# chagmgang/distributed_reinforcement_learning

Measured on AMD Instinct MI355X. Metric: learner env-frames/sec (whole node), IMPALA deep-conv 84x84x4, higher is better.
Workload: dtype bf16; 1 GPU; model=impala deep-conv 84x84x4 + LSTM256 V-trace, global_batch=32, seq_len=20, parallelism=dp1, num_action=18

## Files before the change

distributed_reinforcement_learning_amd/ops/hip/bind.cpp:

```cpp

#include <torch/extension.h>
#include <ATen/hip/HIPContext.h>
#include <hip/hip_runtime.h>

#include <algorithm>
#include <array>
#include <tuple>

#include "drla_kernels.h"

namespace {

hipStream_t cur_stream() {
  return at::hip::getCurrentHIPStream().stream();
}

void check_gpu_contig(const torch::Tensor& t, const char* name) {
  TORCH_CHECK(t.is_cuda(), name, " must be on the GPU");
  TORCH_CHECK(t.is_contiguous(), name, " must be contiguous");
}

template <typename... Ts>
void check_all_gpu_contig(const char* what, const Ts&... ts) {
  (check_gpu_contig(ts, what), ...);
// ... 139 lines not shown
                    slab.scalar_type() == torch::kBFloat16 &&
                    slab.size(0) == batch && slab.size(1) >= row &&
                    slab.stride(1) == 1 && slab.stride(0) >= slab.size(1),
                "out_slab must be a row-major [batch, >= ho*wo*co] bf16 "
                "buffer");
    out_n_stride = slab.stride(0);
    out = slab.as_strided(
        {batch, cfg.ho, cfg.wo, cfg.co},
        {out_n_stride, (long long)cfg.wo * cfg.co, cfg.co, 1});
  } else {
    out = torch::empty({batch, cfg.ho, cfg.wo, cfg.co},
                       in.options().dtype(torch::kBFloat16));
  }
  const dim3 grid(conv_m_tiles(batch * cfg.ho * cfg.wo));
  torch::Tensor x_stash;
  unsigned char* stashp = nullptr;
  if (stash_input) {
    TORCH_CHECK(layer <= 1, "input stash is a u8-layer feature");
    TORCH_CHECK((in.numel() % 16) == 0, "stash wants 16-divisible bytes");
    x_stash = torch::empty_like(in);
    stashp = x_stash.data_ptr<uint8_t>();
  }
  if (layer <= 1) {
    hipLaunchKernelGGL(kConvFwdU8[layer], grid, dim3(DRLA_CONV_BLOCK), 0,
                       cur_stream(), in.data_ptr<uint8_t>(), BF16P(w),
                       BF16P(bias), BF16PM(out), batch, stashp, slotp,
                       in_dist);
  } else {
    hipLaunchKernelGGL(kConvFwdBf16[layer - 2], grid, dim3(DRLA_CONV_BLOCK),
                       0, cur_stream(), BF16P(in), BF16P(w), BF16P(bias),
                       BF16PM(out), batch, out_n_stride);
  }
  return {out, x_stash};
}

static torch::Tensor& dbias_slot_buf(const torch::Tensor& like,
                                     int64_t slot_id) {
  static torch::Tensor bufs[4];
  TORCH_CHECK(slot_id >= 0 && slot_id < 4, "bad slot id");
  if (!bufs[slot_id].defined()) {
    bufs[slot_id] =
        torch::zeros({DRLA_DBIAS_SLOTS * DRLA_DBIAS_STRIDE},
                     like.options().dtype(torch::kFloat));
  }
  return bufs[slot_id];
}

torch::Tensor relu_mask_bwd(torch::Tensor dy, torch::Tensor y, int64_t CO,
                            int64_t slot_id) {
  TORCH_CHECK(dy.is_cuda() && y.is_cuda(), "dy and y must be on GPU");
  TORCH_CHECK(dy.numel() == y.numel() && dy.size(0) == y.size(0),
              "dy and y must hold the same rows");
  long long row_elems = dy.numel() / std::max<int64_t>(dy.size(0), 1);
  auto n_stride_of = [row_elems](const torch::Tensor& t, const char* name) {
    if (t.is_contiguous()) return row_elems;
    for (int d = 1; d < t.dim(); ++d) {
      TORCH_CHECK(t.stride(d - 1) >= t.stride(d), name, " must be row-major");
    }
    TORCH_CHECK(t.stride(t.dim() - 1) == 1 && t.stride(0) >= row_elems &&
                    row_elems % 8 == 0 && t.stride(0) % 8 == 0 &&
                    t.storage_offset() % 8 == 0,
                name, " view must be inner-contiguous and 16 B aligned");
    for (int d = 1; d + 1 < t.dim(); ++d) {
      TORCH_CHECK(t.stride(d) == t.size(d + 1) * t.stride(d + 1), name,
                  " inner dims must be contiguous");
    }
    return (long long)t.stride(0);
  };
  const long long n_stride = n_stride_of(dy, "dy");
  const long long y_n_stride = n_stride_of(y, "y");
  auto out = torch::empty(dy.sizes(), dy.options());
  auto& slots = dbias_slot_buf(dy, slot_id);
  const long long n = dy.numel();
  TORCH_CHECK(n % 8 == 0, "relu_mask_bwd wants numel % 8 == 0");
  int grid = drla_grid(n / 8);
  if (grid > 640) grid = 640;
  hipLaunchKernelGGL(drla_relu_mask_bwd, dim3(grid), dim3(DRLA_BLOCK),
                     0, cur_stream(), BF16P(dy), BF16P(y), BF16PM(out),
                     slots.data_ptr<float>(), n, (int)CO, n_stride,
                     row_elems, y_n_stride);
  return out;
}

std::tuple<torch::Tensor, torch::Tensor> conv_wgrad(int layer,
                                                    torch::Tensor in,
                                                    torch::Tensor dy) {
  check_gpu_contig(in, "in");
  check_gpu_contig(dy, "dy");
  const auto& cfg = conv_layer(layer);
  const int batch = in.size(0);
  const int K = cfg.kh * cfg.kw * cfg.ci;
  static int split_env = [] {
    const char* e = getenv("DRLA_WGRAD_SPLIT");
    return e ? atoi(e) : 0;
  }();
  const int split = split_env ? split_env : ((layer <= 1) ? 512 : 64);
  static torch::Tensor scratch_cache[4];
  if (!scratch_cache[layer].defined()) {
    scratch_cache[layer] =
        torch::zeros({K, cfg.co}, dy.options().dtype(torch::kFloat));
  }
  auto scratch = scratch_cache[layer];
  const dim3 grid((K + DRLA_CONV_WGRAD_BK - 1) / DRLA_CONV_WGRAD_BK, split);
  if (layer <= 1) {
    hipLaunchKernelGGL(kConvWgradU8[layer], grid, dim3(DRLA_CONV_BLOCK), 0,
                       cur_stream(), in.data_ptr<uint8_t>(), BF16P(dy),
                       scratch.data_ptr<float>(), batch);
  } else {
    hipLaunchKernelGGL(kConvWgradBf16[layer - 2], grid,
                       dim3(DRLA_CONV_BLOCK), 0, cur_stream(), BF16P(in),
                       BF16P(dy), scratch.data_ptr<float>(), batch);
  }
  auto dw = torch::empty({cfg.co, K}, dy.options().dtype(torch::kBFloat16));
  auto dbias = torch::empty({cfg.co}, dy.options().dtype(torch::kBFloat16));
  auto& slots = dbias_slot_buf(dy, layer);
  hipLaunchKernelGGL(drla_wgrad_finalize,
                     dim3(drla_grid((long long)K * cfg.co)),
                     dim3(DRLA_BLOCK), 0, cur_stream(),
                     scratch.data_ptr<float>(), BF16PM(dw), K, cfg.co,
                     slots.data_ptr<float>(), BF16PM(dbias));
  return {dw, dbias};
}

torch::Tensor conv_dgrad(int layer, torch::Tensor dy, torch::Tensor w) {
  check_gpu_contig(dy, "dy");
  check_gpu_contig(w, "w");
  TORCH_CHECK(layer == 2 || layer == 3, "dgrad only for l2/l3");
  const auto& cfg = conv_layer(layer);
  const int batch = dy.size(0);
  auto dx = torch::empty({batch, cfg.hi, cfg.wi, cfg.ci},
                         dy.options().dtype(torch::kBFloat16));
  if (layer == 2) {
    const int grid_c = conv_m_tiles(batch * (cfg.hi / 2) * (cfg.wi / 2));
    hipLaunchKernelGGL(drla_conv_dgrad_l2, dim3(grid_c, 4),
                       dim3(DRLA_CONV_BLOCK), 0, cur_stream(), BF16P(dy),
                       BF16P(w), BF16PM(dx), batch);
  } else {
    hipLaunchKernelGGL(drla_conv_dgrad_l3,
                       dim3(conv_m_tiles(batch * cfg.hi * cfg.wi)),
                       dim3(DRLA_CONV_BLOCK), 0, cur_stream(), BF16P(dy),
                       BF16P(w), BF16PM(dx), batch);
  }
  return dx;
}

std::tuple<torch::Tensor, torch::Tensor> dqn_loss_fwd(
    torch::Tensor main_q, torch::Tensor next_main, torch::Tensor next_tgt,
    torch::Tensor actions, torch::Tensor rewards, torch::Tensor discounts,
    torch::Tensor weights) {
  check_all_gpu_contig("dqn_loss input", main_q, next_main, next_tgt,
                       actions, rewards, discounts, weights);
  TORCH_CHECK(actions.scalar_type() == torch::kInt, "actions must be i32");
  const int B = main_q.size(0), A = main_q.size(1);
  const DualPtr mq = dual_ptr(main_q);
  auto fopt = rewards.options().dtype(torch::kFloat);
  auto loss = torch::zeros({1}, fopt);
  auto td = torch::empty({B}, fopt);
  hipLaunchKernelGGL(
      drla_dqn_loss_fwd, dim3((B + 255) / 256), dim3(256), 0, cur_stream(),
      mq.bf16, mq.f32, next_main.data_ptr<float>(), next_tgt.data_ptr<float>(),
      actions.data_ptr<int>(), rewards.data_ptr<float>(),
      discounts.data_ptr<float>(), weights.data_ptr<float>(),
      loss.data_ptr<float>(), td.data_ptr<float>(), B, A);
  return {loss, td};
}

torch::Tensor dqn_loss_bwd(torch::Tensor td, torch::Tensor actions,
                           torch::Tensor weights, torch::Tensor gloss,
                           int64_t A, bool want_bf16) {
  check_all_gpu_contig("dqn_loss bwd input", td, actions, weights, gloss);
  const int B = td.numel();
  auto dmq = torch::empty(
      {B, A},
      td.options().dtype(want_bf16 ? torch::kBFloat16 : torch::kFloat));
  const DualPtr out = dual_ptr(dmq);
  hipLaunchKernelGGL(
      drla_dqn_loss_bwd, dim3(((long long)B * A + 255) / 256), dim3(256), 0,
      cur_stream(), td.data_ptr<float>(), actions.data_ptr<int>(),
      weights.data_ptr<float>(), gloss.data_ptr<float>(), out.bf16, out.f32,
// ... 915 lines not shown
}

void rmsprop_step_t(torch::Tensor p, torch::Tensor g, torch::Tensor ms,
                    double clip, torch::Tensor lr_buf, double rho,
                    double eps) {
  check_all_gpu_contig("rmsprop tensor", p, g, ms, lr_buf);
  const long long n = p.numel();
  torch::Tensor norm_buf;
  if (clip > 0) {
    norm_buf = sq_norm(g);
  } else {
    norm_buf = torch::zeros({1}, p.options());
  }
  hipLaunchKernelGGL(drla_rmsprop_step, dim3(drla_grid(n)), dim3(DRLA_BLOCK),
                     0, cur_stream(), p.data_ptr<float>(),
                     g.data_ptr<float>(), ms.data_ptr<float>(),
                     norm_buf.data_ptr<float>(), static_cast<float>(clip),
                     lr_buf.data_ptr<float>(), static_cast<float>(rho),
                     static_cast<float>(eps), n);
}

void rmsprop_step(torch::Tensor p, torch::Tensor g, torch::Tensor ms,
                  double clip, double lr, double rho, double eps) {
  auto lr_buf = torch::full({1}, lr, p.options());
  rmsprop_step_t(p, g, ms, clip, lr_buf, rho, eps);
}

void adam_step_t(torch::Tensor p, torch::Tensor g, torch::Tensor m,
                 torch::Tensor v, double clip, torch::Tensor lr_buf,
                 double beta1, double beta2, double eps) {
  check_all_gpu_contig("adam tensor", p, g, m, v, lr_buf);
  const long long n = p.numel();
  torch::Tensor norm_buf;
  if (clip > 0) {
    norm_buf = sq_norm(g);
  } else {
    norm_buf = torch::zeros({1}, p.options());
  }
  hipLaunchKernelGGL(drla_adam_step, dim3(drla_grid(n)), dim3(DRLA_BLOCK), 0,
                     cur_stream(), p.data_ptr<float>(), g.data_ptr<float>(),
                     m.data_ptr<float>(), v.data_ptr<float>(),
                     norm_buf.data_ptr<float>(), static_cast<float>(clip),
                     lr_buf.data_ptr<float>(), static_cast<float>(beta1),
                     static_cast<float>(beta2), static_cast<float>(eps), n);
}

void adam_step(torch::Tensor p, torch::Tensor g, torch::Tensor m,
               torch::Tensor v, double clip, double lr_t, double beta1,
               double beta2, double eps) {
  auto lr_buf = torch::full({1}, lr_t, p.options());
  adam_step_t(p, g, m, v, clip, lr_buf, beta1, beta2, eps);
}

}

PYBIND11_MODULE(TORCH_EXTENSION_NAME, m) {
  m.def("normalize_frames_f32", &normalize_frames_f32,
        "uint8 frames -> float32/255 (K11)");
  m.def("normalize_frames_bf16", &normalize_frames_bf16,
        "uint8 frames -> bf16/255 (K11)");
  m.def("vtrace_scan", &vtrace_scan, "fused V-trace reverse scan (K5)");
  m.def("_set_lr_slot", &set_lr_slot,
        "write the learning rate and the input-slot word in one launch");
  m.def("vtrace_loss_fwd", &vtrace_loss_fwd,
        "fused IMPALA loss pipeline forward (K5+K7+K13); nofill: ticketed "
        "fixed-order loss sums, no zero-fill; stash_actions: also returns "
        "a copy of actions made in-kernel",
        py::arg("logits"), py::arg("value"), py::arg("mu"),
        py::arg("actions"), py::arg("rewards"), py::arg("done"),
        py::arg("gamma"), py::arg("clip_mode"), py::arg("c_bl"),
        py::arg("c_ent"), py::arg("nofill") = false,
        py::arg("stash_actions") = false, py::arg("slot") = py::none(),
        py::arg("slot_dist") = std::vector<int64_t>{});
  m.def("vtrace_loss_bwd", &vtrace_loss_bwd,
        "fused IMPALA loss pipeline backward (closed form)");
  m.def("mfma_probe", &mfma_probe, "16x16x32 bf16 MFMA layout probe");
  m.def("conv_fwd", &conv_fwd,
        "MFMA implicit-GEMM conv fwd, fused normalize+bias+ReLU (K1)",
        py::arg("layer"), py::arg("x"), py::arg("w"), py::arg("bias"),
        py::arg("stash_input"), py::arg("out_slab") = py::none(),
        py::arg("slot") = py::none(),
        py::arg("slot_dist") = std::vector<int64_t>{});
  m.def("conv_wgrad", &conv_wgrad, "MFMA conv weight gradient (K1 bwd)");
  m.def("conv_dgrad", &conv_dgrad, "MFMA conv data gradient (K1 bwd)");
  m.def("relu_mask_bwd", &relu_mask_bwd,
        "fused-ReLU backward mask + bias gradient");
  m.def("dqn_loss_fwd", &dqn_loss_fwd,
        "fused double-DQN target + IS-weighted TD loss (K8)");
  m.def("dqn_loss_bwd", &dqn_loss_bwd, "closed-form K8 backward");
  m.def("a2c_loss_fwd", &a2c_loss_fwd, "fused A2C loss fwd (K6)");
  m.def("a2c_loss_bwd", &a2c_loss_bwd, "fused A2C loss bwd (K6)");
  m.def("r2d2_loss_fwd", &r2d2_loss_fwd,
        "fused R2D2 sequence-TD tail fwd (K9; n_step > 1 or "
        "priority_eta >= 0 selects the n-step kernel)",
        py::arg("mq"), py::arg("tq"), py::arg("actions"), py::arg("rewards"),
        py::arg("done"), py::arg("weights"), py::arg("gamma"),
        py::arg("clip_mode"), py::arg("n_step") = 1,
        py::arg("priority_eta") = -1.0);
  m.def("dhead_train_fwd", &dhead_train_fwd,
        "grad-carrying dueling head fwd (R2D2 trained window)");
  m.def("dhead_train_bwd", &dhead_train_bwd,
        "grad-carrying dueling head bwd chain + weight grads");
  m.def("dueling_head_fwd", &dueling_head_fwd,
        "no-grad dueling head over the post-burn-in window");
  m.def("r2d2_loss_bwd", &r2d2_loss_bwd,
        "fused R2D2 sequence-TD tail bwd (K9)");
  m.def("per_update", &per_update, "GPU PER segment-tree batched update");
  m.def("per_sample", &per_sample, "GPU PER stratified sample descent");
  m.def("multi_gather", &multi_gather,
        "one-kernel replay batch gather (all fields)");
  m.def("per_rebuild", &per_rebuild,
        "GPU PER interior-sum rebuild (float32 drift repair)");
  m.def("embed_bwd", &embed_bwd,
        "action-embedding table gradient (K2 backward)");
  m.def("lstm_tail_fwd", &lstm_tail_fwd, "fused LSTM gate tail fwd (K3)",
        py::arg("gates"), py::arg("c_prev"), py::arg("forget_bias"),
        py::arg("stash_c") = false, py::arg("slot") = py::none(),
        py::arg("slot_dist") = std::vector<int64_t>{});
  m.def("lstm_tail_bwd", &lstm_tail_bwd, "fused LSTM gate tail bwd (K3)");
  m.def("mlp_heads_fwd", &mlp_heads_fwd,
        "fused policy+value MLP heads forward (K4)",
        py::arg("h"), py::arg("weights"), py::arg("biases"), py::arg("A"),
        py::arg("want_bwd_bufs") = false);
  m.def("mlp_heads_bwd", &mlp_heads_bwd,
        "fused heads dgrad chain + ReLU masks + bias grads (K4 bwd)",
        py::arg("dlogits"), py::arg("dvalue"), py::arg("stash"),
        py::arg("weights"), py::arg("A"), py::arg("ws") = py::none());
  m.def("embed_mlp_fwd", &embed_mlp_fwd,
        "fused action-embedding MLP forward (K2)",
        py::arg("pa"), py::arg("table"), py::arg("b1"), py::arg("w2"),
        py::arg("b2"), py::arg("stash_idx") = false,
        py::arg("want_w2t") = false, py::arg("xh_slab") = py::none(),
        py::arg("emb_col") = 0, py::arg("h") = py::none(),
        py::arg("slot") = py::none(),
        py::arg("slot_dist") = std::vector<int64_t>{});
  m.def("embed_mlp_bwd", &embed_mlp_bwd,
        "fused action-embedding MLP backward (K2 bwd)",
        py::arg("dy"), py::arg("out"), py::arg("a1"), py::arg("w2"),
        py::arg("idx"), py::arg("A"), py::arg("w2t") = py::none(),
        py::arg("fuse_scatter") = false);
  m.def("mlp_heads_pack_wt", &mlp_heads_pack_wt,
        "one-kernel transposed-weight pack for the heads dgrad");
  m.def("mlp_heads_wgrad", &mlp_heads_wgrad,
        "all six head wgrads (dW = dz^T @ act) in one MFMA launch");
  m.def("lstm_seq_train_fwd", &lstm_seq_train_fwd,
        "grad-carrying whole-sequence LSTM forward (K3 seq, R2D2 train)");
  m.def("lstm_seq_train_bwd", &lstm_seq_train_bwd,
        "whole-sequence LSTM backward (one kernel over the recurrence)");
  m.def("lstm_seq_fwd", &lstm_seq_fwd,
        "whole no-grad LSTM unroll in one kernel (K3 seq / burn-in)");
  m.def("sq_norm", &sq_norm, "squared L2 norm of a flat tensor (K12)");
  m.def("grad_gather", &grad_gather,
        "one-kernel scattered-grad -> flat bucket pack (K12b)");
  m.def("rmsprop_step", &rmsprop_step,
        "fused global-norm-clip + TF-RMSProp update (K12)");
  m.def("rmsprop_step_t", &rmsprop_step_t,
        "RMSProp update with device-tensor lr (hipGraph-safe)");
  m.def("adam_step", &adam_step,
        "fused global-norm-clip + TF-Adam update (K12)");
  m.def("adam_step_t", &adam_step_t,
        "Adam update with device-tensor lr_t (hipGraph-safe)");
  m.def("sq_norm_bf16", &sq_norm_bf16, "squared L2 norm of a bf16 tensor");
  m.def("rmsprop_step_bf16_t", &rmsprop_step_bf16_t,
        "bf16-model/fp32-master RMSProp (K12, mixed precision)");
  m.def("adam_step_bf16_t", &adam_step_bf16_t,
        "bf16-model/fp32-master Adam (K12, mixed precision)");
// ... 2 lines not shown
```

distributed_reinforcement_learning_amd/ops/hip/conv.hip:

```cpp

#include "drla_kernels.h"

#define CONV_KERNEL \
  extern "C" __global__ __launch_bounds__(DRLA_CONV_BLOCK) void

extern "C" __global__ void drla_mfma_probe(const bf16raw* __restrict__ A,
                                           const bf16raw* __restrict__ B,
                                           float* __restrict__ D) {
  const int l = threadIdx.x;
  bf16x8 a_frag, b_frag;
  for (int e = 0; e < 8; ++e) {
    a_frag[e] = (short)A[(l & 15) * 32 + ((l >> 4) * 8 + e)];
    b_frag[e] = (short)B[((l >> 4) * 8 + e) * 16 + (l & 15)];
  }
  f32x4 acc = {0.f, 0.f, 0.f, 0.f};
  acc = __builtin_amdgcn_mfma_f32_16x16x32_bf16(a_frag, b_frag, acc, 0, 0, 0);
  for (int r = 0; r < 4; ++r) {
    D[((l >> 4) * 4 + r) * 16 + (l & 15)] = acc[r];
  }
}


template <typename IN_T, int CI, int CO, int KH, int KW, int STRIDE, int HI,
          int WI, int HO, int WO>
__device__ void conv_fwd_impl(const IN_T* __restrict__ in,
                              const bf16raw* __restrict__ w,
                              const bf16raw* __restrict__ bias,
                              bf16raw* __restrict__ out,
                              int batch,
                              IN_T* __restrict__ x_stash = nullptr,
                              long long out_n_stride = 0) {
  constexpr int K = KH * KW * CI;
  constexpr int BM = DRLA_CONV_BM;
  constexpr int BK = 32;
  constexpr int APAD = 8;
  constexpr int NFRAG = CO / 16;
  const int M = batch * HO * WO;

  __shared__ bf16raw Abuf[BM][BK + APAD];
  __shared__ bf16raw Bbuf[CO][BK + APAD];
  __shared__ float BiasBuf[CO];

  const int tid = threadIdx.x;
  const int wave = tid / 64;
  const int lane = tid % 64;
  const int row0 = blockIdx.x * BM;

  if (tid < CO) BiasBuf[tid] = drla_bf16_to_f32(bias[tid]);

  f32x4 acc[2][NFRAG];
  for (int mi = 0; mi < 2; ++mi)
    for (int ni = 0; ni < NFRAG; ++ni)
      acc[mi][ni] = {0.f, 0.f, 0.f, 0.f};

  const int a_row = tid >> 1;
  const int a_k0 = (tid & 1) * 16;
  const int gm = row0 + a_row;
  const int n_idx = gm / (HO * WO);
  const int rem = gm - n_idx * (HO * WO);
  const int ho = rem / WO;
  const int wo = rem - ho * WO;
  const long long in_base =
      ((long long)n_idx * HI + ho * STRIDE) * WI + wo * STRIDE;

  unsigned int ra4u_0, ra4u_1, ra4u_2, ra4u_3;
  unsigned int ra1u[4];
  bf16x8 rab0 = {0, 0, 0, 0, 0, 0, 0, 0}, rab1 = rab0;
  uint4 rbw4;
  uint2 rbw2;
  constexpr int THREADS_PER_CO = DRLA_CONV_BLOCK / CO;
  constexpr int KCHUNK = BK / THREADS_PER_CO;
  const int b_co = tid / THREADS_PER_CO;
  const int b_kpart = (tid % THREADS_PER_CO) * KCHUNK;

  auto load_chunk = [&](int k0) {
    if (gm < M) {
      if constexpr (CI == 4) {
        const int kk = k0 + a_k0;
        const int kh = kk / (KW * CI);
        const int kw = (kk - kh * KW * CI) / CI;
        const uint4 packed = *reinterpret_cast<const uint4*>(
            in + (in_base + (long long)kh * WI + kw) * CI);
        ra4u_0 = packed.x; ra4u_1 = packed.y;
        ra4u_2 = packed.z; ra4u_3 = packed.w;
// ... 162 lines not shown
    bf16raw* __restrict__ out, float* __restrict__ dbias_slots,
    long long n, int CO, long long n_stride, long long row_elems,
    long long y_n_stride) {
  const long long n8 = n / 8;
  const long long stride = gridDim.x * (long long)blockDim.x;
  long long i = blockIdx.x * (long long)blockDim.x + threadIdx.x;
  const int tid = threadIdx.x;
  float acc[8] = {0, 0, 0, 0, 0, 0, 0, 0};
  const uint4* dy4 = reinterpret_cast<const uint4*>(dy);
  const uint4* y4 = reinterpret_cast<const uint4*>(y);
  uint4* out4 = reinterpret_cast<uint4*>(out);
#define DRLA_RM_LANE(dw, yw, ow, a0, a1)                              \
  {                                                                   \
    const bf16raw d0 = (bf16raw)((dw) & 0xFFFF);                      \
    const bf16raw d1 = (bf16raw)((dw) >> 16);                         \
    const bf16raw m0 =                                                \
        (drla_bf16_to_f32((bf16raw)((yw) & 0xFFFF)) > 0.0f) ? d0 : (bf16raw)0; \
    const bf16raw m1 =                                                \
        (drla_bf16_to_f32((bf16raw)((yw) >> 16)) > 0.0f) ? d1 : (bf16raw)0;    \
    (ow) = ((unsigned int)m1 << 16) | m0;                             \
    (a0) += drla_bf16_to_f32(m0);                                              \
    (a1) += drla_bf16_to_f32(m1);                                              \
  }
  const long long row8 = row_elems / 8;
  const bool strided = (n_stride != row_elems);
  const bool y_strided = (y_n_stride != row_elems);
  for (; i < n8; i += stride) {
    long long si = i, yi = i;
    if (strided || y_strided) {
      const long long r = i / row8;
      const long long c8 = i - r * row8;
      if (strided) si = (r * n_stride) / 8 + c8;
      if (y_strided) yi = (r * y_n_stride) / 8 + c8;
    }
    const uint4 dv = dy4[si];
    const uint4 yv = y4[yi];
    uint4 ov;
    DRLA_RM_LANE(dv.x, yv.x, ov.x, acc[0], acc[1]);
    DRLA_RM_LANE(dv.y, yv.y, ov.y, acc[2], acc[3]);
    DRLA_RM_LANE(dv.z, yv.z, ov.z, acc[4], acc[5]);
    DRLA_RM_LANE(dv.w, yv.w, ov.w, acc[6], acc[7]);
    out4[i] = ov;
  }
#undef DRLA_RM_LANE
  __shared__ float red[DRLA_BLOCK * 8];
  for (int e = 0; e < 8; ++e) red[tid * 8 + e] = acc[e];
  __syncthreads();
  if (tid < CO) {
    const int g = tid / 8;
    const int e = tid % 8;
    float s = 0.0f;
    for (int t = g; t < DRLA_BLOCK; t += CO / 8) s += red[t * 8 + e];
    atomicAdd(&dbias_slots[(blockIdx.x & (DRLA_DBIAS_SLOTS - 1)) *
                               DRLA_DBIAS_STRIDE +
                           tid], s);
  }
}

extern "C" __global__ void drla_wgrad_finalize(
    float* __restrict__ scratch, bf16raw* __restrict__ dw, int K,
    int CO, float* __restrict__ dbias_slots,
    bf16raw* __restrict__ dbias) {
  if (dbias_slots && blockIdx.x == 0 && (int)threadIdx.x < CO) {
    float s = 0.0f;
    for (int t = 0; t < DRLA_DBIAS_SLOTS; ++t) {
      s += dbias_slots[t * DRLA_DBIAS_STRIDE + threadIdx.x];
      dbias_slots[t * DRLA_DBIAS_STRIDE + threadIdx.x] = 0.0f;
    }
    dbias[threadIdx.x] = drla_f32_to_bf16(s);
  }
  long long i = blockIdx.x * (long long)blockDim.x + threadIdx.x;
  const long long total = (long long)K * CO;
  const long long stride = gridDim.x * (long long)blockDim.x;
  for (; i < total; i += stride) {
    const int co = i / K;
    const int k = i - (long long)co * K;
    const long long si = (long long)k * CO + co;
    dw[i] = drla_f32_to_bf16(scratch[si]);
    scratch[si] = 0.0f;
  }
}


template <typename IN_T, int CI, int CO, int KH, int KW, int STRIDE, int HI,
          int WI, int HO, int WO>
__device__ void conv_wgrad_impl(const IN_T* __restrict__ in,
                                const bf16raw* __restrict__ dy,
                                float* __restrict__ scratch,
                                int batch) {
  constexpr int K = KH * KW * CI;
  constexpr int BKM = 64;
  constexpr int BKK = DRLA_CONV_WGRAD_BK;
  constexpr int PAD = 8;
  constexpr int NFRAG = CO / 16;
  constexpr int CO_PER_T = (CO * 32) / DRLA_CONV_BLOCK;
  const int M = batch * HO * WO;

  __shared__ bf16raw Am[2][BKK][BKM + PAD];
  __shared__ bf16raw BmT[2][CO][BKM + PAD];

  const int tid = threadIdx.x;
  const int wave = tid / 64;
  const int lane = tid % 64;
  const int k_row0 = blockIdx.x * BKK;

  f32x4 acc[NFRAG];
  for (int ni = 0; ni < NFRAG; ++ni) acc[ni] = {0.f, 0.f, 0.f, 0.f};

  const int m_per_split = (M + gridDim.y - 1) / gridDim.y;
  const int m_begin = blockIdx.y * m_per_split;
  const int m_end = min(M, m_begin + m_per_split);

  const int a_m = tid >> 2;
  const int a_k = (tid & 3) * 16;
  long long a_off0 = 0, a_off1 = 0;
  long long a_offc[16];
  if constexpr (CI == 4) {
    const int kb = k_row0 + a_k;
    const int kh = kb / (KW * CI);
    a_off0 = (long long)kh * WI + (kb - kh * KW * CI) / CI;
  } else if constexpr (CI == 1) {
    static_assert(K % BKK == 0,
                  "CI==1 contiguous row staging requires K % BKK == 0");
#pragma unroll
    for (int t = 0; t < 16; ++t) {
      const int k2 = k_row0 + a_k + t;
      const int kh = k2 / KW;
      a_offc[t] = (k2 < K) ? (long long)kh * WI + (k2 - kh * KW) : -1;
    }
  } else {
    const int kk0 = k_row0 + a_k;
    const int kh0 = kk0 / (KW * CI);
    const int kwci0 = kk0 - kh0 * KW * CI;
    a_off0 = (kk0 < K)
        ? ((long long)kh0 * WI + kwci0 / CI) * CI + (kwci0 % CI) : -1;
    const int kk1 = kk0 + 8;
    const int kh1 = kk1 / (KW * CI);
    const int kwci1 = kk1 - kh1 * KW * CI;
    a_off1 = (kk1 < K)
        ? ((long long)kh1 * WI + kwci1 / CI) * CI + (kwci1 % CI) : -1;
  }
  const int b_lm0 = tid / (CO / CO_PER_T);
  const int b_co0 = (tid % (CO / CO_PER_T)) * CO_PER_T;

  unsigned int ra4u_0, ra4u_1, ra4u_2, ra4u_3;
  unsigned int ra1u[4];
  bf16x8 rab0 = {0, 0, 0, 0, 0, 0, 0, 0}, rab1 = rab0;
  bf16x8 rb8_0 = rab0, rb8_1 = rab0;
  uint2 rb4_0 = {0, 0}, rb4_1 = {0, 0};
  bool a_live = false, b_live0 = false, b_live1 = false;

  auto load_chunk = [&](int m0) {
    const int m = m0 + a_m;
    a_live = (m < m_end);
    if (a_live) {
      const int n_idx = m / (HO * WO);
      const int rem = m - n_idx * (HO * WO);
      const int ho = rem / WO;
      const int wo = rem - ho * WO;
      const long long base =
          ((long long)n_idx * HI + ho * STRIDE) * WI + wo * STRIDE;
      if constexpr (CI == 4) {
        const uint4 packed = *reinterpret_cast<const uint4*>(
            in + (base + a_off0) * CI);
        ra4u_0 = packed.x; ra4u_1 = packed.y;
        ra4u_2 = packed.z; ra4u_3 = packed.w;
      } else if constexpr (CI == 1) {
#pragma unroll
        for (int rrow = 0; rrow < 2; ++rrow) {
          const unsigned char* src = in + base + a_offc[rrow * 8];
          ra1u[rrow * 2 + 0] = *reinterpret_cast<const unsigned int*>(src);
          ra1u[rrow * 2 + 1] =
              *reinterpret_cast<const unsigned int*>(src + 4);
        }
      } else {
        const bf16raw* inb = reinterpret_cast<const bf16raw*>(in);
        if (a_off0 >= 0) {
          rab0 = *reinterpret_cast<const bf16x8*>(inb + base * CI + a_off0);
        }
        if (a_off1 >= 0) {
          rab1 = *reinterpret_cast<const bf16x8*>(inb + base * CI + a_off1);
        }
      }
    }
    const int mb0 = m0 + b_lm0;
    b_live0 = (mb0 < m_end);
    if (b_live0) {
      if constexpr (CO_PER_T == 8) {
        rb8_0 = *reinterpret_cast<const bf16x8*>(dy + (long long)mb0 * CO +
                                                 b_co0);
      } else {
        rb4_0 = *reinterpret_cast<const uint2*>(dy + (long long)mb0 * CO +
                                                b_co0);
      }
    }
    const int mb1 = m0 + b_lm0 + 32;
    b_live1 = (mb1 < m_end);
    if (b_live1) {
      if constexpr (CO_PER_T == 8) {
        rb8_1 = *reinterpret_cast<const bf16x8*>(dy + (long long)mb1 * CO +
                                                 b_co0);
      } else {
        rb4_1 = *reinterpret_cast<const uint2*>(dy + (long long)mb1 * CO +
                                                b_co0);
      }
    }
  };

  auto store_chunk = [&](int buf) {
    bf16raw (*AmB)[BKM + PAD] = Am[buf];
    bf16raw (*BmTB)[BKM + PAD] = BmT[buf];
    const int lm = a_m;
    if (a_live) {
      if constexpr (CI == 4) {
        const float sc = 1.0f / 255.0f;
#define DRLA_WG_PUT(st, u)                                              \
        {                                                               \
          const int o = a_k + ((st) >> 1) * 8 + ((st) & 1) * 4;         \
          AmB[o + 0][lm] = drla_f32_to_bf16((float)((u) & 0xFF) * sc);  \
          AmB[o + 1][lm] =                                              \
              drla_f32_to_bf16((float)(((u) >> 8) & 0xFF) * sc);        \
          AmB[o + 2][lm] =                                              \
              drla_f32_to_bf16((float)(((u) >> 16) & 0xFF) * sc);       \
          AmB[o + 3][lm] = drla_f32_to_bf16((float)((u) >> 24) * sc);   \
        }
        DRLA_WG_PUT(0, ra4u_0); DRLA_WG_PUT(1, ra4u_1);
        DRLA_WG_PUT(2, ra4u_2); DRLA_WG_PUT(3, ra4u_3);
#undef DRLA_WG_PUT
      } else if constexpr (CI == 1) {
        const float sc1 = 1.0f / 255.0f;
#pragma unroll
        for (int q = 0; q < 4; ++q) {
          const unsigned int u = ra1u[q];
          AmB[a_k + q * 4 + 0][lm] =
              drla_f32_to_bf16((float)(u & 0xFF) * sc1);
          AmB[a_k + q * 4 + 1][lm] =
              drla_f32_to_bf16((float)((u >> 8) & 0xFF) * sc1);
          AmB[a_k + q * 4 + 2][lm] =
              drla_f32_to_bf16((float)((u >> 16) & 0xFF) * sc1);
          AmB[a_k + q * 4 + 3][lm] =
              drla_f32_to_bf16((float)(u >> 24) * sc1);
        }
      } else {
#pragma unroll
        for (int e = 0; e < 8; ++e) {
          AmB[a_k + e][lm] = rab0[e];
          AmB[a_k + 8 + e][lm] = rab1[e];
        }
      }
    } else {
#pragma unroll
      for (int t = 0; t < 16; ++t) AmB[a_k + t][lm] = 0;
    }
    if constexpr (CO_PER_T == 8) {
      const bf16x8 z = {0, 0, 0, 0, 0, 0, 0, 0};
      const bf16x8 v0 = b_live0 ? rb8_0 : z;
      const bf16x8 v1 = b_live1 ? rb8_1 : z;
      const int lm1 = b_lm0 + 32;
#pragma unroll
      for (int e = 0; e < 8; ++e) {
        BmTB[b_co0 + e][b_lm0] = v0[e];
        BmTB[b_co0 + e][lm1] = v1[e];
      }
    } else {
      const uint2 z = {0, 0};
      const uint2 v0 = b_live0 ? rb4_0 : z;
      const uint2 v1 = b_live1 ? rb4_1 : z;
      const int lm1 = b_lm0 + 32;
      BmTB[b_co0 + 0][b_lm0] = (bf16raw)(v0.x & 0xFFFF);
      BmTB[b_co0 + 1][b_lm0] = (bf16raw)(v0.x >> 16);
      BmTB[b_co0 + 2][b_lm0] = (bf16raw)(v0.y & 0xFFFF);
      BmTB[b_co0 + 3][b_lm0] = (bf16raw)(v0.y >> 16);
      BmTB[b_co0 + 0][lm1] = (bf16raw)(v1.x & 0xFFFF);
      BmTB[b_co0 + 1][lm1] = (bf16raw)(v1.x >> 16);
      BmTB[b_co0 + 2][lm1] = (bf16raw)(v1.y & 0xFFFF);
      BmTB[b_co0 + 3][lm1] = (bf16raw)(v1.y >> 16);
    }
  };

  load_chunk(m_begin);
  store_chunk(0);
  load_chunk(m_begin + BKM);
  __syncthreads();
  int nchunks = 0;
  for (int m0 = m_begin; m0 < m_end; m0 += BKM) ++nchunks;
  for (int t = 0; t < nchunks; ++t) {
    const int cur = t & 1;
    if (t + 1 < nchunks) {
      store_chunk(1 - cur);
      load_chunk(m_begin + (long long)(t + 2) * BKM);
    }
    for (int kk = 0; kk < BKM; kk += 32) {
      const bf16x8 a_frag = *reinterpret_cast<const bf16x8*>(
          &Am[cur][wave * 16 + (lane & 15)][kk + (lane >> 4) * 8]);
      for (int ni = 0; ni < NFRAG; ++ni) {
        const int co = ni * 16 + (lane & 15);
        const bf16x8 b_frag = *reinterpret_cast<const bf16x8*>(
            &BmT[cur][co][kk + (lane >> 4) * 8]);
        acc[ni] = __builtin_amdgcn_mfma_f32_16x16x32_bf16(a_frag, b_frag,
                                                          acc[ni], 0, 0, 0);
      }
    }
    __syncthreads();
  }

  for (int ni = 0; ni < NFRAG; ++ni) {
    const int co = ni * 16 + (lane & 15);
    for (int r = 0; r < 4; ++r) {
      const int k = k_row0 + wave * 16 + (lane >> 4) * 4 + r;
      if (k < K) atomicAdd(&scratch[(long long)k * CO + co], acc[ni][r]);
    }
  }
}

CONV_KERNEL drla_conv_wgrad_l1(
    const unsigned char* in, const bf16raw* dy, float* scratch, int batch) {
  conv_wgrad_impl<unsigned char, DRLA_CONV_GEOM(0)>(in, dy, scratch, batch);
}
CONV_KERNEL drla_conv_wgrad_l1_c1(
    const unsigned char* in, const bf16raw* dy, float* scratch, int batch) {
  conv_wgrad_impl<unsigned char, DRLA_CONV_GEOM(1)>(in, dy, scratch, batch);
}
CONV_KERNEL drla_conv_wgrad_l2(
    const bf16raw* in, const bf16raw* dy, float* scratch, int batch) {
  conv_wgrad_impl<bf16raw, DRLA_CONV_GEOM(2)>(in, dy, scratch, batch);
}
CONV_KERNEL drla_conv_wgrad_l3(
    const bf16raw* in, const bf16raw* dy, float* scratch, int batch) {
  conv_wgrad_impl<bf16raw, DRLA_CONV_GEOM(3)>(in, dy, scratch, batch);
}


template <int CI, int CO, int KH, int KW, int STRIDE, int HI, int WI, int HO,
          int WO>
__device__ void conv_dgrad_impl(const bf16raw* __restrict__ dy,
                                const bf16raw* __restrict__ w,
                                bf16raw* __restrict__ dx,
                                int batch) {
  constexpr int K = KH * KW * CI;
  constexpr int Kg = KH * KW * CO;
  constexpr int BM = DRLA_CONV_BM;
  constexpr int BK = 32;
  constexpr int PAD = 8;
  constexpr int NFRAG = CI / 16;
  const int M2 = batch * HI * WI;

  __shared__ bf16raw Ad[BM][BK + PAD];
  __shared__ bf16raw Bd[CI][BK + PAD];

  const int tid = threadIdx.x;
  const int wave = tid / 64;
  const int lane = tid % 64;
  const int row0 = blockIdx.x * BM;

  f32x4 acc[2][NFRAG];
  for (int mi = 0; mi < 2; ++mi)
    for (int ni = 0; ni < NFRAG; ++ni)
      acc[mi][ni] = {0.f, 0.f, 0.f, 0.f};

  const int a_row = tid >> 1;
  const int a_k0 = (tid & 1) * 16;
  const int m2 = row0 + a_row;
  const int n_idx = m2 / (HI * WI);
  const int rem = m2 - n_idx * (HI * WI);
  const int hi = rem / WI;
  const int wi = rem - hi * WI;

  uint4 rda0, rda1;
  bf16raw rbw[8];
  constexpr int CI_PER_T = (CI * BK) / DRLA_CONV_BLOCK;
  const int b_col = tid % BK;
  const int b_ci0 = (tid / BK) * CI_PER_T;

  auto load_chunk = [&](int kg0) {
    const int tap = kg0 / CO;
    const int co0 = kg0 - tap * CO;
    const int kh = tap / KW;
    const int kw = tap - kh * KW;
    bool valid = (m2 < M2);
    int ho = 0, wo = 0;
    if (valid) {
      const int hh = hi - kh;
      const int ww = wi - kw;
      valid = hh >= 0 && ww >= 0 && (hh % STRIDE) == 0 && (ww % STRIDE) == 0;
      if (valid) {
        ho = hh / STRIDE;
        wo = ww / STRIDE;
        valid = ho < HO && wo < WO;
      }
    }
    if (valid) {
      const bf16raw* src =
          dy + ((long long)(n_idx * HO + ho) * WO + wo) * CO + co0 + a_k0;
// ... 178 lines not shown
```

Measured before the change: 1.194 million frames/s.

## Use swizzled row-major LDS tiles with transposed reads in conv wgrad

Rewrites the conv weight-gradient kernel's shared-memory staging. The old kernel scattered per-element transposed stores; the new one writes 16-byte vector chunks into XOR-swizzled row-major tiles and builds MFMA operands with ds_read_tr16_b64 transposed LDS reads. Compile-time checks verify the swizzle is bank-conflict-free and fills every chunk exactly once. It also lowers the default M-split (512→256, 64→48), which trades atomic traffic against parallelism, and adds static asserts that restrict supported shapes.

```diff
diff --git a/distributed_reinforcement_learning_amd/ops/hip/bind.cpp b/distributed_reinforcement_learning_amd/ops/hip/bind.cpp
--- a/distributed_reinforcement_learning_amd/ops/hip/bind.cpp
+++ b/distributed_reinforcement_learning_amd/ops/hip/bind.cpp
@@ -245,6 +245,15 @@
   return out;
 }
 
+int conv_wgrad_split(int layer) {
+  conv_layer(layer);
+  static int split_env = [] {
+    const char* e = getenv("DRLA_WGRAD_SPLIT");
+    return e ? atoi(e) : 0;
+  }();
+  return split_env > 0 ? split_env : ((layer <= 1) ? 256 : 48);
+}
+
 std::tuple<torch::Tensor, torch::Tensor> conv_wgrad(int layer,
                                                     torch::Tensor in,
                                                     torch::Tensor dy) {
@@ -253,11 +262,7 @@
   const auto& cfg = conv_layer(layer);
   const int batch = in.size(0);
   const int K = cfg.kh * cfg.kw * cfg.ci;
-  static int split_env = [] {
-    const char* e = getenv("DRLA_WGRAD_SPLIT");
-    return e ? atoi(e) : 0;
-  }();
-  const int split = split_env ? split_env : ((layer <= 1) ? 512 : 64);
+  const int split = conv_wgrad_split(layer);
   static torch::Tensor scratch_cache[4];
   if (!scratch_cache[layer].defined()) {
     scratch_cache[layer] =
@@ -1339,6 +1344,8 @@
         py::arg("slot") = py::none(),
         py::arg("slot_dist") = std::vector<int64_t>{});
   m.def("conv_wgrad", &conv_wgrad, "MFMA conv weight gradient (K1 bwd)");
+  m.def("_conv_wgrad_split", &conv_wgrad_split,
+        "M-split of the conv wgrad grid for a layer");
   m.def("conv_dgrad", &conv_dgrad, "MFMA conv data gradient (K1 bwd)");
   m.def("relu_mask_bwd", &relu_mask_bwd,
         "fused-ReLU backward mask + bias gradient");
diff --git a/distributed_reinforcement_learning_amd/ops/hip/conv.hip b/distributed_reinforcement_learning_amd/ops/hip/conv.hip
--- a/distributed_reinforcement_learning_amd/ops/hip/conv.hip
+++ b/distributed_reinforcement_learning_amd/ops/hip/conv.hip
@@ -1,5 +1,6 @@
 
 #include "drla_kernels.h"
+#include "conv_wgrad_lds.h"
 
 #define CONV_KERNEL \
   extern "C" __global__ __launch_bounds__(DRLA_CONV_BLOCK) void
@@ -328,6 +329,26 @@
 }
 
 
+__device__ __forceinline__ uint2 drla_u8x4_norm_bf16x4(unsigned int u) {
+  const float sc = 1.0f / 255.0f;
+  uint2 r;
+  r.x = drla_f32x2_to_bf16x2((float)(u & 0xFF) * sc,
+                             (float)((u >> 8) & 0xFF) * sc);
+  r.y = drla_f32x2_to_bf16x2((float)((u >> 16) & 0xFF) * sc,
+                             (float)(u >> 24) * sc);
+  return r;
+}
+
+__device__ __forceinline__ bf16x8 drla_lds_tr_frag(const unsigned char* p,
+                                                   int row_bytes) {
+  typedef __attribute__((ext_vector_type(4))) short s16x4;
+  typedef __attribute__((address_space(3))) s16x4* lds_ptr;
+  const s16x4 lo = __builtin_amdgcn_ds_read_tr16_b64_v4i16((lds_ptr)p);
+  const s16x4 hi =
+      __builtin_amdgcn_ds_read_tr16_b64_v4i16((lds_ptr)(p + 4 * row_bytes));
+  return __builtin_shufflevector(lo, hi, 0, 1, 2, 3, 4, 5, 6, 7);
+}
+
 template <typename IN_T, int CI, int CO, int KH, int KW, int STRIDE, int HI,
           int WI, int HO, int WO>
 __device__ void conv_wgrad_impl(const IN_T* __restrict__ in,
@@ -335,17 +356,26 @@
                                 float* __restrict__ scratch,
                                 int batch) {
   constexpr int K = KH * KW * CI;
-  constexpr int BKM = 64;
+  constexpr int BKM = DRLA_WG_ROWS;
   constexpr int BKK = DRLA_CONV_WGRAD_BK;
-  constexpr int PAD = 8;
   constexpr int NFRAG = CO / 16;
-  constexpr int CO_PER_T = (CO * 32) / DRLA_CONV_BLOCK;
+  constexpr int A_ROWB = BKK * 2;
+  constexpr int B_ROWB = CO * 2;
+  constexpr int B_TPR = CO / 8;
+  constexpr int B_PASSES = BKM * B_TPR / DRLA_CONV_BLOCK;
+  static_assert(K % BKK == 0, "k-blocks are full: no k range checks below");
+  static_assert(BKK == 64 && DRLA_CONV_BLOCK == 256 &&
+                    (B_PASSES == 1 || B_PASSES == 2),
+                "the maps of conv_wgrad_lds.h assume these");
   const int M = batch * HO * WO;
 
-  __shared__ bf16raw Am[2][BKK][BKM + PAD];
-  __shared__ bf16raw BmT[2][CO][BKM + PAD];
+  __shared__ __attribute__((aligned(16))) unsigned char
+      Am[2][BKM * A_ROWB];
+  __shared__ __attribute__((aligned(16))) unsigned char
+      Bm[2][BKM * B_ROWB];
 
   const int tid = threadIdx.x;
+
   const int wave = tid / 64;
   const int lane = tid % 64;
   const int k_row0 = blockIdx.x * BKK;
@@ -386,14 +416,27 @@
     a_off1 = (kk1 < K)
         ? ((long long)kh1 * WI + kwci1 / CI) * CI + (kwci1 % CI) : -1;
   }
-  const int b_lm0 = tid / (CO / CO_PER_T);
-  const int b_co0 = (tid % (CO / CO_PER_T)) * CO_PER_T;
+  const int b_lm0 = drla_wg_b_slot<CO>(tid, 0).row;
+  const int b_ch = drla_wg_b_slot<CO>(tid, 0).ch;
+  const int b_co0 = b_ch * 8;
+  constexpr int B_PASS_ROWS = drla_wg_b_slot<CO>(0, 1).row;
+
+  const int a_st0 = drla_wg_chunk_off<A_ROWB>(drla_wg_a_slot(tid, 0).row,
+                                              drla_wg_a_slot(tid, 0).ch);
+  const int a_st1 = drla_wg_chunk_off<A_ROWB>(drla_wg_a_slot(tid, 1).row,
+                                              drla_wg_a_slot(tid, 1).ch);
+  const int b_st0 = drla_wg_chunk_off<B_ROWB>(b_lm0, b_ch);
+  const int a_rd = drla_wg_tr_off<A_ROWB>(lane, wave);
+  int b_rd[NFRAG];
+#pragma unroll
+  for (int ni = 0; ni < NFRAG; ++ni) {
+    b_rd[ni] = drla_wg_tr_off<B_ROWB>(lane, ni);
+  }
 
   unsigned int ra4u_0, ra4u_1, ra4u_2, ra4u_3;
   unsigned int ra1u[4];
   bf16x8 rab0 = {0, 0, 0, 0, 0, 0, 0, 0}, rab1 = rab0;
   bf16x8 rb8_0 = rab0, rb8_1 = rab0;
-  uint2 rb4_0 = {0, 0}, rb4_1 = {0, 0};
   bool a_live = false, b_live0 = false, b_live1 = false;
 
   auto load_chunk = [&](int m0) {
@@ -432,95 +475,49 @@
     const int mb0 = m0 + b_lm0;
     b_live0 = (mb0 < m_end);
     if (b_live0) {
-      if constexpr (CO_PER_T == 8) {
-        rb8_0 = *reinterpret_cast<const bf16x8*>(dy + (long long)mb0 * CO +
-                                                 b_co0);
-      } else {
-        rb4_0 = *reinterpret_cast<const uint2*>(dy + (long long)mb0 * CO +
-                                                b_co0);
-      }
-    }
-    const int mb1 = m0 + b_lm0 + 32;
-    b_live1 = (mb1 < m_end);
-    if (b_live1) {
-      if constexpr (CO_PER_T == 8) {
+      rb8_0 = *reinterpret_cast<const bf16x8*>(dy + (long long)mb0 * CO +
+                                               b_co0);
+    }
+    if constexpr (B_PASSES == 2) {
+      const int mb1 = m0 + b_lm0 + B_PASS_ROWS;
+      b_live1 = (mb1 < m_end);
+      if (b_live1) {
         rb8_1 = *reinterpret_cast<const bf16x8*>(dy + (long long)mb1 * CO +
                                                  b_co0);
-      } else {
-        rb4_1 = *reinterpret_cast<const uint2*>(dy + (long long)mb1 * CO +
-                                                b_co0);
       }
     }
   };
 
   auto store_chunk = [&](int buf) {
-    bf16raw (*AmB)[BKM + PAD] = Am[buf];
-    bf16raw (*BmTB)[BKM + PAD] = BmT[buf];
-    const int lm = a_m;
+    uint4 a0 = {0, 0, 0, 0}, a1 = {0, 0, 0, 0};
     if (a_live) {
       if constexpr (CI == 4) {
-        const float sc = 1.0f / 255.0f;
-#define DRLA_WG_PUT(st, u)                                              \
-        {                                                               \
-          const int o = a_k + ((st) >> 1) * 8 + ((st) & 1) * 4;         \
-          AmB[o + 0][lm] = drla_f32_to_bf16((float)((u) & 0xFF) * sc);  \
-          AmB[o + 1][lm] =                                              \
-              drla_f32_to_bf16((float)(((u) >> 8) & 0xFF) * sc);        \
-          AmB[o + 2][lm] =                                              \
-              drla_f32_to_bf16((float)(((u) >> 16) & 0xFF) * sc);       \
-          AmB[o + 3][lm] = drla_f32_to_bf16((float)((u) >> 24) * sc);   \
-        }
-        DRLA_WG_PUT(0, ra4u_0); DRLA_WG_PUT(1, ra4u_1);
-        DRLA_WG_PUT(2, ra4u_2); DRLA_WG_PUT(3, ra4u_3);
-#undef DRLA_WG_PUT
+        const uint2 c0 = drla_u8x4_norm_bf16x4(ra4u_0);
+        const uint2 c1 = drla_u8x4_norm_bf16x4(ra4u_1);
+        const uint2 c2 = drla_u8x4_norm_bf16x4(ra4u_2);
+        const uint2 c3 = drla_u8x4_norm_bf16x4(ra4u_3);
+        a0 = {c0.x, c0.y, c1.x, c1.y};
+        a1 = {c2.x, c2.y, c3.x, c3.y};
       } else if constexpr (CI == 1) {
-        const float sc1 = 1.0f / 255.0f;
-#pragma unroll
-        for (int q = 0; q < 4; ++q) {
-          const unsigned int u = ra1u[q];
-          AmB[a_k + q * 4 + 0][lm] =
-              drla_f32_to_bf16((float)(u & 0xFF) * sc1);
-          AmB[a_k + q * 4 + 1][lm] =
-              drla_f32_to_bf16((float)((u >> 8) & 0xFF) * sc1);
-          AmB[a_k + q * 4 + 2][lm] =
-              drla_f32_to_bf16((float)((u >> 16) & 0xFF) * sc1);
-          AmB[a_k + q * 4 + 3][lm] =
-              drla_f32_to_bf16((float)(u >> 24) * sc1);
-        }
+        const uint2 c0 = drla_u8x4_norm_bf16x4(ra1u[0]);
+        const uint2 c1 = drla_u8x4_norm_bf16x4(ra1u[1]);
+        const uint2 c2 = drla_u8x4_norm_bf16x4(ra1u[2]);
+        const uint2 c3 = drla_u8x4_norm_bf16x4(ra1u[3]);
+        a0 = {c0.x, c0.y, c1.x, c1.y};
+        a1 = {c2.x, c2.y, c3.x, c3.y};
       } else {
-#pragma unroll
-        for (int e = 0; e < 8; ++e) {
-          AmB[a_k + e][lm] = rab0[e];
-          AmB[a_k + 8 + e][lm] = rab1[e];
-        }
-      }
-    } else {
-#pragma unroll
-      for (int t = 0; t < 16; ++t) AmB[a_k + t][lm] = 0;
-    }
-    if constexpr (CO_PER_T == 8) {
-      const bf16x8 z = {0, 0, 0, 0, 0, 0, 0, 0};
-      const bf16x8 v0 = b_live0 ? rb8_0 : z;
-      const bf16x8 v1 = b_live1 ? rb8_1 : z;
-      const int lm1 = b_lm0 + 32;
-#pragma unroll
-      for (int e = 0; e < 8; ++e) {
-        BmTB[b_co0 + e][b_lm0] = v0[e];
-        BmTB[b_co0 + e][lm1] = v1[e];
-      }
-    } else {
-      const uint2 z = {0, 0};
-      const uint2 v0 = b_live0 ? rb4_0 : z;
-      const uint2 v1 = b_live1 ? rb4_1 : z;
-      const int lm1 = b_lm0 + 32;
-      BmTB[b_co0 + 0][b_lm0] = (bf16raw)(v0.x & 0xFFFF);
-      BmTB[b_co0 + 1][b_lm0] = (bf16raw)(v0.x >> 16);
-      BmTB[b_co0 + 2][b_lm0] = (bf16raw)(v0.y & 0xFFFF);
-      BmTB[b_co0 + 3][b_lm0] = (bf16raw)(v0.y >> 16);
-      BmTB[b_co0 + 0][lm1] = (bf16raw)(v1.x & 0xFFFF);
-      BmTB[b_co0 + 1][lm1] = (bf16raw)(v1.x >> 16);
-      BmTB[b_co0 + 2][lm1] = (bf16raw)(v1.y & 0xFFFF);
-      BmTB[b_co0 + 3][lm1] = (bf16raw)(v1.y >> 16);
+        a0 = __builtin_bit_cast(uint4, rab0);
+        a1 = __builtin_bit_cast(uint4, rab1);
+      }
+    }
+    *reinterpret_cast<uint4*>(&Am[buf][a_st0]) = a0;
+    *reinterpret_cast<uint4*>(&Am[buf][a_st1]) = a1;
+    const uint4 z = {0, 0, 0, 0};
+    *reinterpret_cast<uint4*>(&Bm[buf][b_st0]) =
+        b_live0 ? __builtin_bit_cast(uint4, rb8_0) : z;
+    if constexpr (B_PASSES == 2) {
+      *reinterpret_cast<uint4*>(&Bm[buf][b_st0 + B_PASS_ROWS * B_ROWB]) =
+          b_live1 ? __builtin_bit_cast(uint4, rb8_1) : z;
     }
   };
 
@@ -536,13 +533,14 @@
       store_chunk(1 - cur);
       load_chunk(m_begin + (long long)(t + 2) * BKM);
     }
+#pragma unroll
     for (int kk = 0; kk < BKM; kk += 32) {
-      const bf16x8 a_frag = *reinterpret_cast<const bf16x8*>(
-          &Am[cur][wave * 16 + (lane & 15)][kk + (lane >> 4) * 8]);
+      const bf16x8 a_frag =
+          drla_lds_tr_frag(&Am[cur][a_rd + kk * A_ROWB], A_ROWB);
+#pragma unroll
       for (int ni = 0; ni < NFRAG; ++ni) {
-        const int co = ni * 16 + (lane & 15);
-        const bf16x8 b_frag = *reinterpret_cast<const bf16x8*>(
-            &BmT[cur][co][kk + (lane >> 4) * 8]);
+        const bf16x8 b_frag =
+            drla_lds_tr_frag(&Bm[cur][b_rd[ni] + kk * B_ROWB], B_ROWB);
         acc[ni] = __builtin_amdgcn_mfma_f32_16x16x32_bf16(a_frag, b_frag,
                                                           acc[ni], 0, 0, 0);
       }
@@ -550,11 +548,13 @@
     __syncthreads();
   }
 
-  for (int ni = 0; ni < NFRAG; ++ni) {
-    const int co = ni * 16 + (lane & 15);
-    for (int r = 0; r < 4; ++r) {
-      const int k = k_row0 + wave * 16 + (lane >> 4) * 4 + r;
-      if (k < K) atomicAdd(&scratch[(long long)k * CO + co], acc[ni][r]);
+  if (nchunks > 0) {
+    for (int ni = 0; ni < NFRAG; ++ni) {
+      const int co = ni * 16 + (lane & 15);
+      for (int r = 0; r < 4; ++r) {
+        const int k = k_row0 + wave * 16 + (lane >> 4) * 4 + r;
+        atomicAdd(&scratch[(long long)k * CO + co], acc[ni][r]);
+      }
     }
   }
 }
diff --git a/distributed_reinforcement_learning_amd/ops/hip/conv_wgrad_lds.h b/distributed_reinforcement_learning_amd/ops/hip/conv_wgrad_lds.h
--- /dev/null
+++ b/distributed_reinforcement_learning_amd/ops/hip/conv_wgrad_lds.h
@@ -0,0 +1,115 @@
+#pragma once
+
+#define DRLA_WG_ROWS 64
+
+template <int ROWB>
+constexpr int drla_wg_swizzle(int row) {
+  static_assert(ROWB == 64 || ROWB == 128, "tile rows are 64 or 128 bytes");
+  return ROWB == 128
+             ? ((row & 1) | (((row >> 1) & 1) << 1) | (((row >> 3) & 1) << 2))
+             : (((row >> 3) & 1) << 1);
+}
+
+template <int ROWB>
+constexpr int drla_wg_chunk_off(int row, int ch) {
+  return ROWB * row + 16 * (ch ^ drla_wg_swizzle<ROWB>(row));
+}
+
+template <int ROWB>
+constexpr int drla_wg_elem_off(int row, int col) {
+  return drla_wg_chunk_off<ROWB>(row, col >> 3) + 2 * (col & 7);
+}
+
+template <int ROWB>
+constexpr int drla_wg_tr_off(int lane, int tile) {
+  const int g = lane >> 4, q = (lane >> 2) & 3, p = lane & 3;
+  return drla_wg_chunk_off<ROWB>(8 * g + q, 2 * tile + (p >> 1)) + 8 * (p & 1);
+}
+
+struct DrlaWgSlot { int row, ch; };
+constexpr DrlaWgSlot drla_wg_a_slot(int tid, int j) {
+  return {tid >> 2, 2 * (tid & 3) + j};
+}
+template <int CO>
+constexpr DrlaWgSlot drla_wg_b_slot(int tid, int j) {
+  return {tid / (CO / 8) + j * (256 / (CO / 8)), tid % (CO / 8)};
+}
+
+
+template <int ROWB>
+constexpr bool drla_wg_gather_ok() {
+  for (int tile = 0; tile < ROWB / 32; ++tile)
+    for (int ks = 0; ks < 2; ++ks)
+      for (int h = 0; h < 2; ++h)
+        for (int lane = 0; lane < 64; ++lane) {
+          const int g = lane >> 4, i = lane & 15;
+          if (drla_wg_tr_off<ROWB>(lane, tile) % 8) return false;
+          for (int q = 0; q < 4; ++q) {
+            const int src = 16 * g + 4 * q + (i >> 2);
+            const int got = drla_wg_tr_off<ROWB>(src, tile) +
+                            (32 * ks + 4 * h) * ROWB + 2 * (i & 3);
+            const int want = drla_wg_elem_off<ROWB>(
+                32 * ks + 8 * g + 4 * h + q, 16 * tile + i);
+            if (got != want) return false;
+          }
+        }
+  return true;
+}
+
+template <int ROWB>
+constexpr bool drla_wg_reads_conflict_free() {
+  for (int tile = 0; tile < ROWB / 32; ++tile)
+    for (int step = 0; step < 4; ++step)
+      for (int half = 0; half < 2; ++half) {
+        bool used[64] = {};
+        for (int l = 0; l < 32; ++l) {
+          const int a = drla_wg_tr_off<ROWB>(32 * half + l, tile) +
+                        (32 * (step >> 1) + 4 * (step & 1)) * ROWB;
+          for (int d = 0; d < 2; ++d) {
+            const int bank = (a / 4 + d) % 64;
+            if (used[bank]) return false;
+            used[bank] = true;
+          }
+        }
+      }
+  return true;
+}
+
+template <int ROWB, typename SlotFn>
+constexpr bool drla_wg_stores_ok(SlotFn slot, int passes) {
+  bool filled[DRLA_WG_ROWS * ROWB / 16] = {};
+  for (int j = 0; j < passes; ++j)
+    for (int grp = 0; grp < 32; ++grp) {
+      bool used[32] = {};
+      for (int l = 0; l < 8; ++l) {
+        const DrlaWgSlot s = slot(8 * grp + l, j);
+        if (s.row < 0 || s.row >= DRLA_WG_ROWS || s.ch < 0 ||
+            s.ch >= ROWB / 16)
+          return false;
+        const int a = drla_wg_chunk_off<ROWB>(s.row, s.ch);
+        if (a % 16 || a < 0 || a >= DRLA_WG_ROWS * ROWB) return false;
+        if (filled[a / 16]) return false;
+        filled[a / 16] = true;
+        for (int d = 0; d < 4; ++d) {
+          const int bank = (a / 4 + d) % 32;
+          if (used[bank]) return false;
+          used[bank] = true;
+        }
+      }
+    }
+  for (int c = 0; c < DRLA_WG_ROWS * ROWB / 16; ++c)
+    if (!filled[c]) return false;
+  return true;
+}
+
+static_assert(drla_wg_gather_ok<128>() && drla_wg_gather_ok<64>(),
+              "transposed reads must deliver the 16x16x32 operand map");
+static_assert(drla_wg_reads_conflict_free<128>() &&
+                  drla_wg_reads_conflict_free<64>(),
+              "transposed reads must be bank-conflict-free");
+static_assert(drla_wg_stores_ok<128>(drla_wg_a_slot, 2),
+              "A tile stores: conflict-free, every chunk once");
+static_assert(drla_wg_stores_ok<128>(drla_wg_b_slot<64>, 2),
+              "dY tile stores (CO=64): conflict-free, every chunk once");
+static_assert(drla_wg_stores_ok<64>(drla_wg_b_slot<32>, 1),
+              "dY tile stores (CO=32): conflict-free, every chunk once");
```

After: 1.249 million frames/s (median of 6 runs). +4.6%, better.
